# vitskvara/VBMatrixFactorization.jl

Hardware: AMD Instinct MI355X
Metric: VB iterations/sec (higher is better)
Workload: dtype bf16

## Files before the change

### include/vbmf_hip.h

```cpp
#ifndef VBMF_HIP_H
#define VBMF_HIP_H

#include <stddef.h>
#include <stdint.h>

#ifdef __cplusplus
extern "C" {
#endif

typedef struct vbmf_ctx vbmf_ctx;

typedef enum {
    VBMF_OK = 0,
    VBMF_ERR_INVALID = -1,
    VBMF_ERR_NO_DEVICE = -2,
    VBMF_ERR_HIP = -3,
    VBMF_ERR_NUMERIC = -4,
    VBMF_ERR_COMM = -5,
    VBMF_ERR_UNSUPPORTED = -6,
    VBMF_ERR_SYNC = -7
} vbmf_status;

#define VBMF_Y_F32 0
#define VBMF_Y_BF16 1
// ... 192 lines not shown
int vbmf_dual_set_priors(vbmf_ctx* ctx, int64_t H0, double alpha00, double beta00, double alpha01, double beta01,
                         double alpha0, double alpha1);
int vbmf_dual_get_priors(vbmf_ctx* ctx, int64_t* H0, double* priors6);
int vbmf_dual_run(vbmf_ctx* ctx, int64_t niter, double eps, int est_cb, int est_priors, int64_t* iters_done,
                  double* d_last, double* trace);

int vbmf_trial_set_priors(vbmf_ctx* ctx, int64_t H0, int64_t M0, const double* priors9);
int vbmf_trial_get_priors(vbmf_ctx* ctx, int64_t* H0, int64_t* M0, double* priors9);
int vbmf_trial_run(vbmf_ctx* ctx, int64_t niter, double eps, int est_cb, int est_priors, int64_t* iters_done,
                   double* d_last, double* trace);


typedef struct vbmf_prep vbmf_prep;
int vbmf_preprocess_open(vbmf_prep** out, int device, const double* Y, int64_t L, int64_t M, int64_t ldY, int64_t* L_used);
int vbmf_preprocess_rows(const vbmf_prep* plan, int64_t* used_rows0, double* mu, double* den);
int vbmf_set_Y_preprocessed(vbmf_ctx* ctx, const vbmf_prep* plan, double lambda);
int vbmf_preprocess_close(vbmf_prep* plan);

#define VBMF_UNIQUE_ID_BYTES 128
int vbmf_comm_unique_id(void* id128);
int vbmf_comm_init(vbmf_ctx* ctx, const void* id128);
typedef int (*vbmf_allreduce_fn)(void* user, void* buf, size_t count, int is_double, void* hip_stream);
int vbmf_comm_set_transport(vbmf_ctx* ctx, vbmf_allreduce_fn fn, void* user);

int vbmf_profile_enable(vbmf_ctx* ctx, int on);
int vbmf_profile_read(vbmf_ctx* ctx, double* out8, int reset);
int vbmf_pass_bytes(vbmf_ctx* ctx, int pass, double* bytes);
int vbmf_device_sync(vbmf_ctx* ctx);

#define VBMF_PEEK_P 0
#define VBMF_PEEK_Q 1
#define VBMF_PEEK_A32 2
#define VBMF_PEEK_B32 3
#define VBMF_PEEK_FA 4
#define VBMF_PEEK_FB 5
#define VBMF_PEEK_Y1 6
#define VBMF_PEEK_Y2 7
#define VBMF_PEEK_DIMS 8
#define VBMF_PEEK_CHAIN 9
#define VBMF_PEEK_STATE 10
#define VBMF_PEEK_GRAM_W 11
#define VBMF_PEEK_GRAM_PQ 12
#define VBMF_PEEK_GRAM_G 13
#define VBMF_PEEK_SA32 14
#define VBMF_PEEK_SB32 15
int vbmf_debug_peek(vbmf_ctx* ctx, int what, uint32_t* out, int64_t nwords, int64_t word_offset);
int vbmf_debug_time_pass(vbmf_ctx* ctx, int pass, int iters, double* ms);
#define VBMF_DEBUG_EPI_SPIN_LIMIT 0
#define VBMF_DEBUG_EPI_EXPECT_SKEW 1
#define VBMF_DEBUG_SIGMA_B_PPM 2
#define VBMF_DEBUG_EXACT_LAMBDA 3
int vbmf_debug_set(vbmf_ctx* ctx, int what, int64_t value);
int vbmf_debug_lambda_max(vbmf_ctx* ctx, const double* G, double* lambda_max, double* kernel_us);

#ifdef __cplusplus
}
#endif
#endif
```

### vbmatrixfactorization.jl_amd/capi.py

```python
import ctypes as C
import os

import numpy as np

_HERE = os.path.dirname(os.path.abspath(__file__))
LIB_PATH = os.environ.get("VBMF_HIP_LIB") or os.path.join(_HERE, "libvbmf_hip.so")
if os.environ.get("VBMF_HIP_LIB") and not os.path.isfile(LIB_PATH):
    raise FileNotFoundError(f"VBMF_HIP_LIB={LIB_PATH}: no such library (A/B variant builds: scripts/README.md)")

VBMF_Y_F32, VBMF_Y_BF16 = 0, 1
VBMF_SRC_F64, VBMF_SRC_F32, VBMF_SRC_BF16 = 0, 1, 2
VBMF_DST_F64, VBMF_DST_F32, VBMF_DST_BF16 = 0, 1, 2
VBMF_OUT_YHAT, VBMF_OUT_RESIDUAL = 0, 1
VBMF_FACTOR_A, VBMF_FACTOR_B = 0, 1
VBMF_FACTOR_AUTO, VBMF_FACTOR_BF16, VBMF_FACTOR_BF16X2 = 0, 1, 2
VBMF_FACTOR_BF16_MAX_H = 128
VBMF_VARIANT_BASIC, VBMF_VARIANT_SPARSE_DIAG, VBMF_VARIANT_SPARSE_DIAGVAR, VBMF_VARIANT_DUAL_DIAG, VBMF_VARIANT_TRIAL_DIAG = 0, 1, 2, 3, 4
VBMF_VARIANT_DUAL_DIAGVAR, VBMF_VARIANT_TRIAL_DIAGVAR = 5, 6
VBMF_COMPAT_SPECTRAL_DELTA, VBMF_COMPAT_SPARSE_REPEAT, VBMF_COMPAT_DEFAULT = 1, 2, 0xFFFFFFFF
STEP_A, STEP_B, STEP_CA, STEP_CB, STEP_SIGMA2 = 1, 2, 4, 8, 16
UNIQUE_ID_BYTES = 128
VBMF_FIT_FORM_STREAM, VBMF_FIT_FORM_GRAM, VBMF_FIT_FORM_AUTO = 0, 1, 2
VBMF_FIT_GRAM_WIDE_FACTOR = 2
VBMF_FIT_LDS_CAP_BYTES = 144 * 1024
# ... 10 lines not shown
        raise ValueError(f"form = {form!r} ('stream', 'gram' or 'auto')")
    return FIT_FORMS[form]


def ard_fit_form_code(form):
    if form == "gram":
        raise ValueError("form = 'gram': the ARD-sparse, two-group and three-group models have no Gram form (the element-wise precision "
                         "on A breaks A = Y'V); it serves the basic model's wide bags through vbmf_batch_")
    if not isinstance(form, str) or form not in ARD_FIT_FORMS:
        raise ValueError(f"form = {form!r} ('stream', 'split' or 'auto')")
    return ARD_FIT_FORMS[form]


def ard_slice_cols(slice_cols):
    sc = 0 if slice_cols is None else int(slice_cols)
    if sc != 0 and (sc < 8 or sc % 8):
        raise ValueError(f"slice_cols = {slice_cols!r} (None, or a multiple of 8)")
    return sc


def ard_fit_slices(Mb, slice_cols=None):
    sc = ard_slice_cols(slice_cols) or VBMF_FIT_SPLIT_COLS
    return -(-int(Mb) // sc)


def ard_fit_form_auto(Mb, full_cov=False):
    return VBMF_FIT_FORM_SPLIT if Mb >= (VBMF_FIT_SPLIT_MIN_COLS_FULL if full_cov else VBMF_FIT_SPLIT_MIN_COLS) else VBMF_FIT_FORM_STREAM


def fit_gram_fits(L, H):
    P = 16 if H <= 16 else 32
    return 3 * L * H <= VBMF_FIT_LDS_CAP_BYTES // 8 - (P * (P + 2) + 9 * H * H)


def fit_form_auto(L, Mb, H):
    return int(Mb >= VBMF_FIT_GRAM_WIDE_FACTOR * L and fit_gram_fits(L, H))

SYMBOLS = [
    "vbmf_default_opts", "vbmf_create", "vbmf_destroy", "vbmf_last_error", "vbmf_set_Y", "vbmf_set_Y_rows", "vbmf_set_Y_synthetic",
    "vbmf_get_Y", "vbmf_get_trYY", "vbmf_set_state", "vbmf_get_state", "vbmf_step", "vbmf_run", "vbmf_run_fixed_basis",
    "vbmf_run_fixed_basis_batched", "vbmf_fit_batched", "vbmf_fit_batched_form", "vbmf_bags_row_gram", "vbmf_get_YHat",
    "vbmf_elbo", "vbmf_comm_unique_id", "vbmf_comm_init", "vbmf_comm_set_transport", "vbmf_profile_enable", "vbmf_profile_read",
    "vbmf_pass_bytes", "vbmf_device_sync", "vbmf_debug_peek", "vbmf_debug_time_pass", "vbmf_debug_lambda_max",
    "vbmf_sparse_set_state", "vbmf_sparse_get_state", "vbmf_sparse_step", "vbmf_sparse_run", "vbmf_sparse_run_fixed_basis",
    "vbmf_sparse_run_fixed_basis_batched", "vbmf_sparse_fit_batched", "vbmf_local_fit_batched", "vbmf_rows_fit_batched",
    "vbmf_ard_fit_batched_form",
    "vbmf_sparse_lower_bound", "vbmf_sparse_set_noise_rows", "vbmf_sparse_get_noise_rows", "vbmf_preprocess_open", "vbmf_preprocess_rows", "vbmf_set_Y_preprocessed",
    "vbmf_preprocess_close", "vbmf_dual_set_priors", "vbmf_dual_get_priors", "vbmf_dual_run",
    "vbmf_trial_set_priors", "vbmf_trial_get_priors", "vbmf_trial_run",
    "vbmf_sparse_set_full_cov", "vbmf_sparse_set_SigmaA", "vbmf_sparse_get_SigmaA",
    "vbmf_sparse_lower_bound_trimmed", "vbmf_debug_set",
    "vbmf_bag_residuals", "vbmf_sparse_lower_bound_batched", "vbmf_bag_least_squares", "vbmf_bag_least_squares_jobs", "vbmf_set_gram_form",
    "vbmf_sparse_fixed_basis_jobs", "vbmf_debug_vbls_jobs_lds_cols",
    "vbmf_get_YHat_rows", "vbmf_get_factor_rows", "vbmf_set_Y_gather",
]
VBMF_OK, VBMF_ERR_INVALID, VBMF_ERR_NO_DEVICE, VBMF_ERR_HIP, VBMF_ERR_NUMERIC, VBMF_ERR_COMM, VBMF_ERR_UNSUPPORTED, VBMF_ERR_SYNC = 0, -1, -2, -3, -4, -5, -6, -7
DEBUG_EPI_SPIN_LIMIT, DEBUG_EPI_EXPECT_SKEW, DEBUG_SIGMA_B_PPM, DEBUG_EXACT_LAMBDA = 0, 1, 2, 3
SSTEP_A, SSTEP_B, SSTEP_CA, SSTEP_CB, SSTEP_SIGMA, SSTEP_PRIORS = 1, 2, 4, 8, 16, 32
(PEEK_P, PEEK_Q, PEEK_A32, PEEK_B32, PEEK_FA, PEEK_FB, PEEK_Y1, PEEK_Y2, PEEK_DIMS, PEEK_CHAIN, PEEK_STATE, PEEK_GRAM_W,
 PEEK_GRAM_PQ, PEEK_GRAM_G, PEEK_SA32, PEEK_SB32) = range(16)


class VbmfOpts(C.Structure):
    _fields_ = [
        ("struct_size", C.c_int32), ("device", C.c_int32), ("y_dtype", C.c_int32), ("factor_dtype", C.c_int32),
        ("variant", C.c_int32), ("reference_compat", C.c_uint32), ("nranks", C.c_int32), ("rank", C.c_int32),
        ("L_global", C.c_int64), ("row_offset", C.c_int64), ("pass1_splits", C.c_int32), ("reserved", C.c_int32),
    ]


class VbmfSparseHyper(C.Structure):
    _fields_ = [("alpha0", C.c_double), ("beta0", C.c_double), ("gamma0", C.c_double), ("delta0", C.c_double),
                ("eta0", C.c_double), ("zeta0", C.c_double)]


ALLREDUCE_FN = C.CFUNCTYPE(C.c_int, C.c_void_p, C.c_void_p, C.c_size_t, C.c_int, C.c_void_p)


class VbmfError(RuntimeError):
    def __init__(self, code, msg):
        super().__init__(f"vbmf_hip error {code}: {msg}")
        self.code = code


_lib = None


def lib():
    global _lib
    if _lib is not None:
        return _lib
    try:
        import torch
    except Exception:
        pass
    if not os.path.exists(LIB_PATH):
        raise ImportError(
            f"{LIB_PATH} is missing: build it with `python vbmatrixfactorization.jl_amd/build.py` "
            "(hipcc, gfx950).  This package has no CPU fallback.")
    L = C.CDLL(LIB_PATH, mode=C.RTLD_GLOBAL)
    dp, i64, i32, vp = C.POINTER(C.c_double), C.c_int64, C.c_int, C.c_void_p
    L.vbmf_default_opts.argtypes = [C.POINTER(VbmfOpts)]
    L.vbmf_default_opts.restype = None
    L.vbmf_create.argtypes = [C.POINTER(vp), i64, i64, i64, C.POINTER(VbmfOpts)]
    L.vbmf_destroy.argtypes = [vp]
    L.vbmf_last_error.argtypes = [vp]
    L.vbmf_last_error.restype = C.c_char_p
# ... 1 lines not shown
    L.vbmf_set_Y_rows.argtypes = [vp, vp, C.c_int32, C.c_int32, i64, i64, i64, i64]
    L.vbmf_set_Y_gather.argtypes = [vp, vp, C.POINTER(i64), i64]
    L.vbmf_set_Y_synthetic.argtypes = [vp, C.c_uint64, i64, C.c_double]
    L.vbmf_get_Y.argtypes = [vp, dp, i64, i64, i64]
    L.vbmf_get_trYY.argtypes = [vp, dp]
    L.vbmf_set_state.argtypes = [vp, dp, i64, dp, i64, dp, dp, dp, dp, C.c_double, C.POINTER(i64), i64, i64]
    L.vbmf_get_state.argtypes = [vp, dp, i64, dp, i64, dp, dp, dp, dp, dp]
    L.vbmf_step.argtypes = [vp, i32]
    L.vbmf_run.argtypes = [vp, i64, C.c_double, i32, i32, C.POINTER(i64), dp, dp]
    L.vbmf_run_fixed_basis.argtypes = [vp, i64]
    L.vbmf_run_fixed_basis_batched.argtypes = [vp, i64, C.POINTER(i64), i64, dp, dp, dp, dp, i64]
    L.vbmf_fit_batched.argtypes = ([vp, i64, C.POINTER(i64), i64, C.POINTER(i64), i64, C.c_double, i32, i32] + [dp] * 7
                                   + [C.POINTER(i64), dp, C.POINTER(i64), dp])
    L.vbmf_fit_batched_form.argtypes = L.vbmf_fit_batched.argtypes + [i64, C.POINTER(i64)]
    L.vbmf_bags_row_gram.argtypes = [vp, i64, C.POINTER(i64), dp]
    L.vbmf_sparse_run_fixed_basis.argtypes = [vp, i64]
    L.vbmf_sparse_run_fixed_basis_batched.argtypes = [vp, i64, C.POINTER(i64), i64, i32, dp, dp, dp, dp, dp, dp, dp, dp, dp, dp, dp]
    L.vbmf_sparse_fit_batched.argtypes = ([vp, i64, C.POINTER(i64), i64, C.POINTER(i64), i64, C.c_double, i32, i32, i32, i64] + [dp] * 16
                                          + [C.POINTER(i64), dp, C.POINTER(i64), dp])
    L.vbmf_local_fit_batched.argtypes = ([vp, i64, C.POINTER(i64), i64, C.POINTER(i64), i64, C.c_double, i32, i32, i32, i64,
                                          C.POINTER(i64), i64] + [dp] * 16 + [C.POINTER(i64), dp, C.POINTER(i64), dp])
    L.vbmf_rows_fit_batched.argtypes = L.vbmf_local_fit_batched.argtypes
    L.vbmf_ard_fit_batched_form.argtypes = L.vbmf_local_fit_batched.argtypes + [C.c_int, i64, i64, C.POINTER(i64)]
    L.vbmf_get_YHat.argtypes = [vp, dp, i64]
    L.vbmf_get_YHat_rows.argtypes = [vp, C.c_int32, vp, C.c_int32, C.c_int32, i64, i64, i64, i64]
    L.vbmf_get_factor_rows.argtypes = [vp, C.c_int32, vp, C.c_int32, C.c_int32, i64, i64, i64, i64]
    L.vbmf_elbo.argtypes = [vp, dp]
    L.vbmf_comm_unique_id.argtypes = [vp]
    L.vbmf_comm_init.argtypes = [vp, vp]
    L.vbmf_comm_set_transport.argtypes = [vp, ALLREDUCE_FN, vp]
    L.vbmf_profile_enable.argtypes = [vp, i32]
    L.vbmf_profile_read.argtypes = [vp, dp, i32]
    L.vbmf_pass_bytes.argtypes = [vp, i32, dp]
    L.vbmf_device_sync.argtypes = [vp]
    L.vbmf_debug_peek.argtypes = [vp, i32, C.POINTER(C.c_uint32), i64, i64]
    L.vbmf_debug_time_pass.argtypes = [vp, i32, i32, dp]
    L.vbmf_debug_lambda_max.argtypes = [vp, dp, dp, dp]
    L.vbmf_sparse_set_state.argtypes = [vp, dp, dp, dp, dp, dp, i64, dp, dp, dp, C.c_double, C.c_double,
                                        C.POINTER(VbmfSparseHyper), C.POINTER(i64), i64, i64]
    L.vbmf_sparse_get_state.argtypes = [vp, dp, dp, dp, dp, dp, dp, i64, dp, dp, dp, dp, dp]
    L.vbmf_sparse_step.argtypes = [vp, i32]
    L.vbmf_sparse_run.argtypes = [vp, i64, C.c_double, i32, C.POINTER(i64), dp, dp]
    L.vbmf_sparse_lower_bound.argtypes = [vp, i32, dp]
    L.vbmf_sparse_lower_bound_trimmed.argtypes = [vp, i32, C.c_double, dp]
    L.vbmf_debug_set.argtypes = [vp, i32, i64]
    L.vbmf_bag_residuals.argtypes = [vp, i64, C.POINTER(i64), dp, i64, dp]
    L.vbmf_sparse_lower_bound_batched.argtypes = [vp, i64, C.POINTER(i64), i32, C.c_double, i32] + [dp] * 15
    L.vbmf_bag_least_squares.argtypes = [vp, i64, C.POINTER(i64), dp, i64, i64, C.c_double, dp, i64, dp]
    L.vbmf_bag_least_squares_jobs.argtypes = [vp, i64, C.POINTER(i64), i64, C.POINTER(i64), dp, dp, i64, C.POINTER(i64), C.POINTER(i64), dp, dp,
                                              C.POINTER(i64)]
    L.vbmf_sparse_fixed_basis_jobs.argtypes = [vp, i64, C.POINTER(i64), i64, i64, i32, i64, dp, dp, dp, dp, dp, dp, dp, dp, i64,
                                               C.POINTER(i64), C.POINTER(i64), dp, dp, dp, dp, dp, dp, dp, dp, C.POINTER(i64)]
    L.vbmf_debug_vbls_jobs_lds_cols.argtypes = [i64, i32]
    L.vbmf_sparse_set_full_cov.argtypes = [vp, i32]
    L.vbmf_set_gram_form.argtypes = [vp, i32]
    L.vbmf_sparse_set_SigmaA.argtypes = [vp, dp]
    L.vbmf_sparse_get_SigmaA.argtypes = [vp, dp]
    L.vbmf_dual_set_priors.argtypes = [vp, i64] + [C.c_double] * 6
    L.vbmf_dual_get_priors.argtypes = [vp, C.POINTER(i64), dp]
    L.vbmf_dual_run.argtypes = [vp, i64, C.c_double, i32, i32, C.POINTER(i64), dp, dp]
    L.vbmf_trial_set_priors.argtypes = [vp, i64, i64, dp]
    L.vbmf_trial_get_priors.argtypes = [vp, C.POINTER(i64), C.POINTER(i64), dp]
    L.vbmf_trial_run.argtypes = [vp, i64, C.c_double, i32, i32, C.POINTER(i64), dp, dp]
    L.vbmf_sparse_set_noise_rows.argtypes = [vp, dp, dp, C.c_double]
    L.vbmf_sparse_get_noise_rows.argtypes = [vp, dp, dp]
    L.vbmf_preprocess_open.argtypes = [C.POINTER(vp), i32, dp, i64, i64, i64, C.POINTER(i64)]
    L.vbmf_preprocess_rows.argtypes = [vp, C.POINTER(i64), dp, dp]
    L.vbmf_set_Y_preprocessed.argtypes = [vp, vp, C.c_double]
    L.vbmf_preprocess_close.argtypes = [vp]
    for name in SYMBOLS:
        if name not in ("vbmf_default_opts", "vbmf_last_error"):
            getattr(L, name).restype = C.c_int
    _lib = L
    return L


def _dptr(a):
    return a.ctypes.data_as(C.POINTER(C.c_double)) if a is not None else None


def _i64ptr(a):
    return a.ctypes.data_as(C.POINTER(C.c_int64)) if a is not None else None


def _fcol(a, shape=None):
    a = np.asarray(a, dtype=np.float64)
    if shape is not None and tuple(a.shape) != tuple(shape):
        raise ValueError(f"expected shape {shape}, got {a.shape}")
    return np.asfortranarray(a)


def _is_tensor(a):
    return hasattr(a, "data_ptr") and hasattr(a, "is_cuda")


def y_source(src, device=0):
    if _is_tensor(src):
        import torch
        codes = {torch.float64: VBMF_SRC_F64, torch.float32: VBMF_SRC_F32, torch.bfloat16: VBMF_SRC_BF16}
        if src.dtype not in codes:
            raise TypeError(f"Y must be float64, float32 or bfloat16, got {src.dtype}")
        if src.dim() != 2:
            raise ValueError("Y must be a matrix")
        if src.is_cuda:
            if src.device.index != device:
                raise ValueError(f"Y lives on {src.device}, the context on GPU {device}")
# ... 662 lines not shown
        out = np.zeros(8)
        self._chk(self._lib.vbmf_profile_read(self._h, _dptr(out), int(reset)))
        return dict(pass1_ms=out[0], pass1_n=int(out[1]), pass2_ms=out[2], pass2_n=int(out[3]))

    def pass_bytes(self, p):
        v = C.c_double()
        self._chk(self._lib.vbmf_pass_bytes(self._h, p, C.byref(v)))
        return v.value

    def peek(self, what, nwords, offset=0, dtype=np.uint32):
        out = np.zeros(nwords, dtype=np.uint32)
        self._chk(self._lib.vbmf_debug_peek(self._h, what, out.ctypes.data_as(C.POINTER(C.c_uint32)), nwords, offset))
        return out.view(dtype)

    def chain_us(self):
        v = self.peek(PEEK_CHAIN, 16, dtype=np.uint64)
        return dict(zip(("ctrl_end", "SigmaA", "lambda_max_dB_and_loop", "SigmaB", "epilogue_table", "epilogue_tiles", "epilogue_fold"),
                        (float(x) * 0.01 for x in v)))

    def dims(self):
        v = self.peek(PEEK_DIMS, 30, dtype=np.int32)
        keys = ["Hp", "NH", "mode", "XT1", "KS1", "nsplit1", "sps1", "XT2", "KS2", "nsplit2", "sps2", "kstep", "npart", "narrow",
                "streamk_per", "streamk_grid",
                "gram", "gram_built", "gram_build_us", "gram_nsplit",
                "p_frag", "q_frag", "q_epi",
                "lds8", "xcd_map", "post3",
                "sparse_a_fused",
                "set_y_rows_us",
                "b_pending", "b_materialised"]
        return dict(zip(keys, (int(x) for x in v)))

    def out_rows_us(self):
        return int(self.peek(PEEK_DIMS, 31, dtype=np.int32)[30])

    def time_pass(self, p, iters=10):
        v = C.c_double()
        self._chk(self._lib.vbmf_debug_time_pass(self._h, p, iters, C.byref(v)))
        return v.value

    def lambda_max(self, G):
        G = np.asfortranarray(G, dtype=np.float64)
        assert G.shape == (self.H, self.H)
        v, us = C.c_double(), C.c_double()
        self._chk(self._lib.vbmf_debug_lambda_max(self._h, _dptr(G), C.byref(v), C.byref(us)))
        return v.value, us.value

    def sync(self):
        self._chk(self._lib.vbmf_device_sync(self._h))

    def debug_set(self, what, value):
        self._chk(self._lib.vbmf_debug_set(self._h, int(what), int(value)))


def vbls_jobs_lds_cols(H, full_cov=False):
    return int(lib().vbmf_debug_vbls_jobs_lds_cols(int(H), int(bool(full_cov))))
```

### vbmatrixfactorization.jl_amd/csrc/blk_inverse.hpp

```cpp
#pragma once
#include "common.hpp"

namespace vbmf {

typedef __attribute__((ext_vector_type(4))) double f64x4;

__device__ __forceinline__ double blk_rcp(double x) {
    double r = __builtin_amdgcn_rcp(x);
    r = fma(fma(-x, r, 1.0), r, r);
    r = fma(fma(-x, r, 1.0), r, r);
    return r;
}

template <int K>
__device__ __forceinline__ double row_bcast16(double v) {
    const int lo = __builtin_amdgcn_mov_dpp(__double2loint(v), 0x150 + K, 0xf, 0xf, false);
    const int hi = __builtin_amdgcn_mov_dpp(__double2hiint(v), 0x150 + K, 0xf, 0xf, false);
    return __hiloint2double(hi, lo);
}
template <int Q0>
__device__ __forceinline__ unsigned rows_bcast_u32(unsigned x) {
    const auto p = __builtin_amdgcn_permlane16_swap(x, x, false, false);
    const unsigned y = (Q0 & 1) ? p[1] : p[0];
    const auto s = __builtin_amdgcn_permlane32_swap(y, y, false, false);
// ... 41 lines not shown
    if constexpr (KK < 15) un = bperm_f64(rowaddr[Q1], a[R1]);
    double v[4];
#pragma unroll
    for (int r = 0; r < 4; ++r) v[r] = row_bcast16<KK>(a[r]);
    const double d = row_bcast16<KK>(u);
    pv.push(d);
    if (pivout != nullptr && c == 0 && q == 0) pivout[KK] = d;
    const double dinv = blk_rcp(d);
    const bool is_col = (c == KK), is_row = (q == Q0);
    const double w = is_col ? -dinv : u * dinv;
    v[R0] = is_row ? -1.0 : v[R0];
#pragma unroll
    for (int r = 0; r < 4; ++r) a[r] = fma(-v[r], w, zero_if(is_col || (r == R0 && is_row), a[r]));
    if constexpr (KK < 15) {
        const double vk1 = row_bcast16<KK>(un);
        u = fma(-vk1, w, zero_if(is_col, un));
    }
}
__device__ __forceinline__ void sweep16(f64x4& a, int lane, PivAcc& pv, double* pivout = nullptr) {
    const int c = lane & 15, q = lane >> 4;
    const int rowaddr[4] = {4 * c, 4 * (16 + c), 4 * (32 + c), 4 * (48 + c)};
    double u = bperm_f64(rowaddr[0], a[0]);
    sweep16_step<0>(a, u, c, q, rowaddr, pv, pivout);  sweep16_step<1>(a, u, c, q, rowaddr, pv, pivout);  sweep16_step<2>(a, u, c, q, rowaddr, pv, pivout);
    sweep16_step<3>(a, u, c, q, rowaddr, pv, pivout);  sweep16_step<4>(a, u, c, q, rowaddr, pv, pivout);  sweep16_step<5>(a, u, c, q, rowaddr, pv, pivout);
    sweep16_step<6>(a, u, c, q, rowaddr, pv, pivout);  sweep16_step<7>(a, u, c, q, rowaddr, pv, pivout);  sweep16_step<8>(a, u, c, q, rowaddr, pv, pivout);
    sweep16_step<9>(a, u, c, q, rowaddr, pv, pivout);  sweep16_step<10>(a, u, c, q, rowaddr, pv, pivout); sweep16_step<11>(a, u, c, q, rowaddr, pv, pivout);
    sweep16_step<12>(a, u, c, q, rowaddr, pv, pivout); sweep16_step<13>(a, u, c, q, rowaddr, pv, pivout); sweep16_step<14>(a, u, c, q, rowaddr, pv, pivout);
    sweep16_step<15>(a, u, c, q, rowaddr, pv, pivout);
    pv.fold();
}

__device__ __forceinline__ f64x4 blk_ld_rows(const double* W, int ld, int bi, int bj, int lane) {
    const double* p = W + (16 * bi + (lane >> 4)) * ld + 16 * bj + (lane & 15);
    return f64x4{p[0], p[4 * ld], p[8 * ld], p[12 * ld]};
}
__device__ __forceinline__ f64x4 blk_ld_cols(const double* W, int ld, int bi, int bj, int lane) {
    const double* p = W + (16 * bi + (lane & 15)) * ld + 16 * bj + (lane >> 4);
    return f64x4{p[0], p[4], p[8], p[12]};
}
__device__ __forceinline__ void blk_st_rows(double* W, int ld, int bi, int bj, int lane, const f64x4& x) {
    double* p = W + (16 * bi + (lane >> 4)) * ld + 16 * bj + (lane & 15);
    p[0] = x[0]; p[4 * ld] = x[1]; p[8 * ld] = x[2]; p[12 * ld] = x[3];
}
__device__ __forceinline__ void blk_st_cols(double* W, int ld, int bi, int bj, int lane, const f64x4& x) {
    double* p = W + (16 * bi + (lane & 15)) * ld + 16 * bj + (lane >> 4);
    p[0] = x[0]; p[4] = x[1]; p[8] = x[2]; p[12] = x[3];
}
__device__ __forceinline__ f64x4 blk_mma(const f64x4& a, const f64x4& b, f64x4 acc) {
#pragma unroll
    for (int kk = 0; kk < 4; ++kk) acc = __builtin_amdgcn_mfma_f64_16x16x4f64(a[kk], b[kk], acc, 0, 0, 0);
    return acc;
}

template <int NB, int NW>
__device__ __forceinline__ void blk_sweep(double* W, int ld, int nb_used, int w, int lane, PivAcc& pv) {
    for (int K = 0; K < nb_used; ++K) {
        f64x4 S = blk_ld_rows(W, ld, K, K, lane);
        sweep16(S, lane, pv);
        const f64x4 Sn = -S;
        f64x4 R[NB];
#pragma unroll
        for (int J = 0; J < NB; ++J) {
            if (J >= nb_used || J == K) continue;
            const f64x4 b = J > K ? blk_ld_rows(W, ld, K, J, lane) : blk_ld_cols(W, ld, J, K, lane);
            R[J] = blk_mma(Sn, b, f64x4{0.0, 0.0, 0.0, 0.0});
        }
        int pairno = 0;
#pragma unroll
        for (int I = 0; I < NB; ++I) {
            if (I >= nb_used || I == K) continue;
            f64x4 T = I < K ? blk_ld_cols(W, ld, I, K, lane) : blk_ld_rows(W, ld, K, I, lane);
            T = -T;
#pragma unroll
            for (int J = I; J < NB; ++J) {
                if (J >= nb_used || J == K) continue;
                if (NW == 1 || (pairno % NW) == w) {
                    f64x4 C = blk_ld_rows(W, ld, I, J, lane);
                    C = blk_mma(T, R[J], C);
                    blk_st_rows(W, ld, I, J, lane, C);
                }
                ++pairno;
            }
        }
        if constexpr (NW > 1) __syncthreads();
        if (NW == 1 || w == 0) {
#pragma unroll
            for (int J = 0; J < NB; ++J) {
                if (J >= nb_used || J == K) continue;
                if (J > K) blk_st_rows(W, ld, K, J, lane, R[J]);
                else blk_st_cols(W, ld, J, K, lane, R[J]);
            }
            blk_st_rows(W, ld, K, K, lane, S);
        }
        if constexpr (NW > 1) __syncthreads();
    }
}

constexpr int INV256_LD = 258;
constexpr int INV256_LDS_DOUBLES = 2 * 16 * INV256_LD + 16 * 18;
__device__ __forceinline__ void inv256_blk(const double* __restrict__ Kg, double* __restrict__ Out, double* lds, double* pivs, int nb = 16) {
    constexpr int LD = INV256_LD, NBLK = 136, NOWN = 9;
    double* Tst = lds;
    double* Rst = lds + 16 * LD;
    double* Sb = lds + 2 * 16 * LD;
    const int lane = threadIdx.x & 63;
    const int w = __builtin_amdgcn_readfirstlane(threadIdx.x >> 6);
    int bi[NOWN], bj[NOWN];
    f64x4 blk[NOWN];
// ... 7 lines not shown
        bj[t] = have ? I + (p - start) : -1;
        blk[t] = f64x4{0.0, 0.0, 0.0, 0.0};
        if (have) blk[t] = blk_ld_rows(Kg, 256, bi[t], bj[t], lane);
    }
    for (int K = 0; K < nb; ++K) {
#pragma unroll
        for (int t = 0; t < NOWN; ++t) {
            if (bi[t] < 0) continue;
            if (bi[t] == K && bj[t] == K) {
                PivAcc pv;
                sweep16(blk[t], lane, pv, pivs + 16 * K);
                blk_st_rows(Sb, 18, 0, 0, lane, -blk[t]);
            } else if (bi[t] == K) {
                blk_st_rows(Tst, LD, 0, bj[t], lane, blk[t]);
            } else if (bj[t] == K) {
                blk_st_cols(Tst, LD, 0, bi[t], lane, blk[t]);
            }
        }
        __syncthreads();
        const f64x4 Sn = blk_ld_rows(Sb, 18, 0, 0, lane);
#pragma unroll
        for (int t = 0; t < NOWN; ++t) {
            if (bi[t] < 0 || (bi[t] == K) == (bj[t] == K)) continue;
            const int J = bi[t] == K ? bj[t] : bi[t];
            const f64x4 b = blk_ld_rows(Tst, LD, 0, J, lane);
            const f64x4 R = blk_mma(Sn, b, f64x4{0.0, 0.0, 0.0, 0.0});
            blk_st_rows(Rst, LD, 0, J, lane, R);
            if (bi[t] == K) blk[t] = R;
        }
        __syncthreads();
#pragma unroll
        for (int t = 0; t < NOWN; ++t) {
            if (bi[t] < 0) continue;
            if (bi[t] != K && bj[t] != K) {
                const f64x4 T = -blk_ld_rows(Tst, LD, 0, bi[t], lane);
                const f64x4 Rj = blk_ld_rows(Rst, LD, 0, bj[t], lane);
                blk[t] = blk_mma(T, Rj, blk[t]);
            } else if (bj[t] == K && bi[t] != K) {
                blk[t] = blk_ld_cols(Rst, LD, 0, bi[t], lane);
            }
        }
        __syncthreads();
    }
#pragma unroll
    for (int t = 0; t < NOWN; ++t) {
        if (bi[t] < 0) continue;
        const f64x4 v = -blk[t];
        blk_st_rows(Out, 256, bi[t], bj[t], lane, v);
        if (bi[t] != bj[t]) blk_st_cols(Out, 256, bj[t], bi[t], lane, v);
    }
    __syncthreads();
}

}
```

### vbmatrixfactorization.jl_amd/csrc/vbmf_hip.hip

```cpp
#include "../../include/vbmf_hip.h"

#include <hip/hip_runtime.h>
#include <rccl/rccl.h>

#include <algorithm>
#include <chrono>
#include <cmath>
#include <cstdio>
#include <cstring>
#include <string>
#include <thread>
#include <type_traits>
#include <vector>

#include "common.hpp"
#include "ctx_cache.hpp"
#include "ctx_mem.hpp"
#include "ctrl_kernels.hpp"
#include "post_kernels.hpp"
#include "rng.hpp"
#include "sparse_kernels.hpp"
#include "stream_gemm.hpp"
#include "tile_kernels.hpp"
#include "prep_kernels.hpp"
// ... 2135 lines not shown
    HIPCHK(c, hipGetLastError());
    return VBMF_OK;
}
static int launch_yhat_out(vbmf_ctx* c, int what, void* dev, int dt, int64_t l0, int64_t n, int64_t rs, int64_t cs) {
    if (dt == VBMF_DST_F64) return launch_yhat_typed<double, double>(c, what, (double*)dev, l0, n, rs, cs);
    if (dt == VBMF_DST_F32) return launch_yhat_typed<float, float>(c, what, (float*)dev, l0, n, rs, cs);
    return launch_yhat_typed<float, out_bf16>(c, what, (out_bf16*)dev, l0, n, rs, cs);
}
static int launch_factor_out(vbmf_ctx* c, const float* F, void* dev, int dt, int64_t x0, int64_t n, int64_t rs, int64_t cs) {
    const int grid = grid_for(n * c->H), hfast = cs <= rs;
#define VBMF_FAC_LAUNCH(T)                                                                                                  \
    hipLaunchKernelGGL((factor_out_kernel<T>), dim3(grid), dim3(256), 0, c->stream, F, c->Hp, (int)c->H, (long long)x0, \
                       (long long)n, (T*)dev, (long long)rs, (long long)cs, hfast)
    if (dt == VBMF_DST_F64) VBMF_FAC_LAUNCH(double);
    else if (dt == VBMF_DST_F32) VBMF_FAC_LAUNCH(float);
    else VBMF_FAC_LAUNCH(out_bf16);
#undef VBMF_FAC_LAUNCH
    HIPCHK(c, hipGetLastError());
    return VBMF_OK;
}

template <class Emit>
static int write_block(vbmf_ctx* c, const char* fn, void* dst, int dt, int on_device, int64_t row0, int64_t nrows, int64_t ncols,
                       int64_t rs, int64_t cs, Emit emit) {
    const size_t es = dst_elem_size(dt);
    if (!c->ev_y[0]) { HIPCHK(c, hipEventCreate(&c->ev_y[0])); HIPCHK(c, hipEventCreate(&c->ev_y[1])); }
    HIPCHK(c, hipEventRecord(c->ev_y[0], c->stream));
    if (on_device) {
        TRY(emit(dst, row0, nrows, rs, cs));
    } else {
        const bool rowmajor = cs == 1 && (nrows == 1 || rs >= ncols);
        int64_t rc = std::max<int64_t>(1, (int64_t)(256ll << 20) / (ncols * (int64_t)es));
        rc = std::min(rc, nrows);
        DevScratch<void> stage;
        MEMCHK(c, stage.alloc((size_t)rc * ncols * es));
        for (int64_t r = 0; r < nrows; r += rc) {
            const int64_t n = std::min(rc, nrows - r);
            TRY(rowmajor ? emit(stage.get(), row0 + r, n, ncols, (int64_t)1) : emit(stage.get(), row0 + r, n, (int64_t)1, n));
            char* to = (char*)dst + (size_t)r * rs * es;
            hipError_t e = rowmajor ? hipMemcpy2DAsync(to, (size_t)rs * es, stage, (size_t)ncols * es, (size_t)ncols * es, (size_t)n, hipMemcpyDeviceToHost, c->stream)
                                    : hipMemcpy2DAsync(to, (size_t)cs * es, stage, (size_t)n * es, (size_t)n * es, (size_t)ncols, hipMemcpyDeviceToHost, c->stream);
            if (e == hipSuccess) e = hipStreamSynchronize(c->stream);
            if (e != hipSuccess) FAIL(c, VBMF_ERR_HIP, "%s: copy to the host failed: %s", fn, hipGetErrorString(e));
        }
    }
    HIPCHK(c, hipEventRecord(c->ev_y[1], c->stream));
    HIPCHK(c, hipStreamSynchronize(c->stream));
    float ms = 0.0f;
    HIPCHK(c, hipEventElapsedTime(&ms, c->ev_y[0], c->ev_y[1]));
    c->out_ms = ms;
    return VBMF_OK;
}

extern "C" {

int vbmf_get_YHat_rows(vbmf_ctx* c, int32_t what, void* dst, int32_t dt, int32_t on_device, int64_t row0, int64_t nrows,
                       int64_t rs, int64_t cs) {
    if (!c) return VBMF_ERR_INVALID;
    static const char* fn = "vbmf_get_YHat_rows";
    if (!dst) FAIL(c, VBMF_ERR_INVALID, "%s: null dst", fn);
    if (what != VBMF_OUT_YHAT && what != VBMF_OUT_RESIDUAL) FAIL(c, VBMF_ERR_INVALID, "%s: unknown what %d", fn, (int)what);
    TRY(check_dst(c, fn, dst, dt, on_device, row0, nrows, c->L, c->M, rs, cs));
    if (!c->cache.have_state()) FAIL(c, VBMF_ERR_INVALID, "%s: no state", fn);
    if (what == VBMF_OUT_RESIDUAL && !c->cache.have_Y()) FAIL(c, VBMF_ERR_INVALID, "%s: no Y", fn);
    TRY(ensure_B(c));
    TRY(rebuild_B32_if_stale(c));
    return write_block(c, fn, dst, dt, on_device, row0, nrows, c->M, rs, cs,
                       [&](void* dev, int64_t l0, int64_t n, int64_t r, int64_t s) { return launch_yhat_out(c, what, dev, dt, l0, n, r, s); });
}

int vbmf_get_factor_rows(vbmf_ctx* c, int32_t which, void* dst, int32_t dt, int32_t on_device, int64_t row0, int64_t nrows,
                         int64_t rs, int64_t cs) {
    if (!c) return VBMF_ERR_INVALID;
    static const char* fn = "vbmf_get_factor_rows";
    if (!dst) FAIL(c, VBMF_ERR_INVALID, "%s: null dst", fn);
    if (which != VBMF_FACTOR_A && which != VBMF_FACTOR_B) FAIL(c, VBMF_ERR_INVALID, "%s: unknown which %d", fn, (int)which);
    TRY(check_dst(c, fn, dst, dt, on_device, row0, nrows, which == VBMF_FACTOR_A ? c->M : c->L, c->H, rs, cs));
    if (!c->cache.have_state()) FAIL(c, VBMF_ERR_INVALID, "%s: no state", fn);
    if (which == VBMF_FACTOR_B) {
        TRY(ensure_B(c));
        TRY(rebuild_B32_if_stale(c));
    }
    return write_block(c, fn, dst, dt, on_device, row0, nrows, c->H, rs, cs, [&](void* dev, int64_t x0, int64_t n, int64_t r, int64_t s) {
        return launch_factor_out(c, which == VBMF_FACTOR_A ? c->A32 : c->B32[c->bcur], dev, dt, x0, n, r, s);
    });
}

int vbmf_elbo(vbmf_ctx* c, double* elbo) {
    if (!c || !elbo) return VBMF_ERR_INVALID;
    HIPCHK(c, hipSetDevice(c->o.device));
    TRY(ensure_ready(c));
    TRY(ensure_gram_A(c));
    TRY(ensure_gram_B(c));
    int f = 0;
    TRY(prepare_trYBA(c, &f));
    TRY(launch_ctrl_end(c, f, 0.0, nullptr));
    HIPCHK(c, hipMemcpyAsync(c->scal_host, c->st + c->lay.scal(), 32 * 8, hipMemcpyDeviceToHost, c->stream));
    HIPCHK(c, hipStreamSynchronize(c->stream));
    *elbo = c->scal_host[S_ELBO];
    return VBMF_OK;
}

int vbmf_comm_unique_id(void* id128) {
    if (!id128) return VBMF_ERR_INVALID;
    static_assert(sizeof(ncclUniqueId) <= VBMF_UNIQUE_ID_BYTES, "unique id size");
    ncclUniqueId id;
// ... 111 lines not shown
}

int vbmf_debug_time_pass(vbmf_ctx* c, int pass, int iters, double* ms) {
    if (!c || !ms || (pass != 1 && pass != 2) || iters < 1) return VBMF_ERR_INVALID;
    HIPCHK(c, hipSetDevice(c->o.device));
    TRY(ensure_ready(c));
    hipEvent_t a, b;
    HIPCHK(c, hipEventCreate(&a));
    HIPCHK(c, hipEventCreate(&b));
    const int prof = c->prof;
    c->prof = 0;
    int rc = launch_stream(c, pass - 1);
    if (rc == VBMF_OK) rc = launch_stream(c, pass - 1);
    hipEventRecord(a, c->stream);
    for (int i = 0; i < iters && rc == VBMF_OK; ++i) rc = launch_stream(c, pass - 1);
    hipEventRecord(b, c->stream);
    hipEventSynchronize(b);
    float t = 0.f;
    hipEventElapsedTime(&t, a, b);
    hipEventDestroy(a);
    hipEventDestroy(b);
    c->prof = prof;
    c->cache.P_overwritten();
    *ms = t / iters;
    return rc;
}

int vbmf_debug_lambda_max(vbmf_ctx* c, const double* G, double* lam, double* kernel_us) {
    if (!c || !G || !lam) return VBMF_ERR_INVALID;
    HIPCHK(c, hipSetDevice(c->o.device));
    TRY(ensure_B(c));
    const int H = (int)c->H, Hp = c->Hp;
    std::vector<double> g((size_t)Hp * Hp, 0.0);
    for (int j = 0; j < H; ++j)
        for (int i = 0; i < H; ++i) g[(size_t)i * Hp + j] = G[(size_t)j * H + i];
    HIPCHK(c, hipMemcpyAsync(c->st + c->lay.GD(), g.data(), g.size() * sizeof(double), hipMemcpyHostToDevice, c->stream));
    HIPCHK(c, hipMemsetAsync(c->ints + I_STOP, 0, sizeof(int), c->stream));
    hipEvent_t a, b;
    HIPCHK(c, hipEventCreate(&a));
    HIPCHK(c, hipEventCreate(&b));
    hipEventRecord(a, c->stream);
    int rc = launch_eig(c, 1, 0);
    hipEventRecord(b, c->stream);
    hipEventSynchronize(b);
    float t = 0.f;
    hipEventElapsedTime(&t, a, b);
    hipEventDestroy(a);
    hipEventDestroy(b);
    if (rc != VBMF_OK) return rc;
    HIPCHK(c, hipMemcpyAsync(lam, c->st + c->lay.scal() + S_LAMD, sizeof(double), hipMemcpyDeviceToHost, c->stream));
    HIPCHK(c, hipStreamSynchronize(c->stream));
    if (kernel_us) *kernel_us = 1e3 * (double)t;
    return VBMF_OK;
}

int vbmf_debug_set(vbmf_ctx* c, int what, int64_t value) {
    if (!c) return VBMF_ERR_INVALID;
    HIPCHK(c, hipSetDevice(c->o.device));
    TRY(ensure_B(c));
    switch (what) {
        case VBMF_DEBUG_EXACT_LAMBDA:
            c->exact_lambda = value != 0;
            return VBMF_OK;
        case VBMF_DEBUG_EPI_SPIN_LIMIT:
            if (value < 1 || value > (1ll << 30)) FAIL(c, VBMF_ERR_INVALID, "vbmf_debug_set: spin limit out of range");
            c->epi_spin_limit = (int)value;
            return VBMF_OK;
        case VBMF_DEBUG_EPI_EXPECT_SKEW:
            c->epi_expect_skew = value ? 1 : 0;
            return VBMF_OK;
        case VBMF_DEBUG_SIGMA_B_PPM: {
            if (value < -1000000 || value > 1000000) FAIL(c, VBMF_ERR_INVALID, "vbmf_debug_set: ppm out of range");
            c->dbg_sb_ppm = (int)value;
            HIPCHK(c, hipSetDevice(c->o.device));
            HIPCHK(c, memcpy_sync(c, c->ints + I_DBG_SB_PPM, &c->dbg_sb_ppm, sizeof(int), hipMemcpyHostToDevice));
            return VBMF_OK;
        }
        default: FAIL(c, VBMF_ERR_INVALID, "vbmf_debug_set: unknown knob");
    }
}

int vbmf_device_sync(vbmf_ctx* c) {
    if (!c) return VBMF_ERR_INVALID;
    HIPCHK(c, hipSetDevice(c->o.device));
    HIPCHK(c, hipStreamSynchronize(c->stream));
    return VBMF_OK;
}


}

static double digamma_host(double x) {
    double r = 0.0;
    while (x < 10.0) { r -= 1.0 / x; x += 1.0; }
    const double f = 1.0 / (x * x);
    return r + std::log(x) - 0.5 / x -
           f * (1.0 / 12 - f * (1.0 / 120 - f * (1.0 / 252 - f * (1.0 / 240 - f * (5.0 / 660 - f * (691.0 / 32760))))));
}

static int launch_sparse_cov_b(vbmf_ctx* c) {
    ctrl_tier(c->H, [&](auto r, auto t) {
        constexpr int R = decltype(r)::value, T = decltype(t)::value;
        hipLaunchKernelGGL((sparse_cov_b_kernel<R, T>), dim3(1), dim3(T * T), (cov_lds_bytes<R, T>()), ctrl_stream(c), c->st, c->lay, (int)c->H,
                           c->SB32, c->ints, c->diagvar ? 1 : 0);
    });
    HIPCHK(c, hipGetLastError());
// ... 780 lines not shown
```

Baseline: 4741.

## Add look-ahead blocked sweep overlapping next pivot with bulk updates

For small block counts with multiple waves, the blocked sweep inverse now dedicates one wave to the critical path: it sweeps the diagonal block and precomputes the next pivot block early. The remaining waves perform the trailing Schur updates in parallel. This aims to shorten the serialized pivot chain per block step, at the cost of more complex mirror-indexing logic and extra barriers on the last step. A debug entry point for testing the sweep in isolation is also added.

```diff
diff --git a/include/vbmf_hip.h b/include/vbmf_hip.h
--- a/include/vbmf_hip.h
+++ b/include/vbmf_hip.h
@@ -268,6 +268,7 @@
 #define VBMF_DEBUG_EXACT_LAMBDA 3
 int vbmf_debug_set(vbmf_ctx* ctx, int what, int64_t value);
 int vbmf_debug_lambda_max(vbmf_ctx* ctx, const double* G, double* lambda_max, double* kernel_us);
+int vbmf_debug_blk_sweep(const double* K, int64_t H, int waves, double* out, double* logdet, int* bad);
 
 #ifdef __cplusplus
 }
diff --git a/vbmatrixfactorization.jl_amd/capi.py b/vbmatrixfactorization.jl_amd/capi.py
--- a/vbmatrixfactorization.jl_amd/capi.py
+++ b/vbmatrixfactorization.jl_amd/capi.py
@@ -86,7 +86,7 @@
     "vbmf_sparse_lower_bound_trimmed", "vbmf_debug_set",
     "vbmf_bag_residuals", "vbmf_sparse_lower_bound_batched", "vbmf_bag_least_squares", "vbmf_bag_least_squares_jobs", "vbmf_set_gram_form",
     "vbmf_sparse_fixed_basis_jobs", "vbmf_debug_vbls_jobs_lds_cols",
-    "vbmf_get_YHat_rows", "vbmf_get_factor_rows", "vbmf_set_Y_gather",
+    "vbmf_get_YHat_rows", "vbmf_get_factor_rows", "vbmf_set_Y_gather", "vbmf_debug_blk_sweep",
 ]
 VBMF_OK, VBMF_ERR_INVALID, VBMF_ERR_NO_DEVICE, VBMF_ERR_HIP, VBMF_ERR_NUMERIC, VBMF_ERR_COMM, VBMF_ERR_UNSUPPORTED, VBMF_ERR_SYNC = 0, -1, -2, -3, -4, -5, -6, -7
 DEBUG_EPI_SPIN_LIMIT, DEBUG_EPI_EXPECT_SKEW, DEBUG_SIGMA_B_PPM, DEBUG_EXACT_LAMBDA = 0, 1, 2, 3
@@ -194,6 +194,7 @@
     L.vbmf_sparse_fixed_basis_jobs.argtypes = [vp, i64, C.POINTER(i64), i64, i64, i32, i64, dp, dp, dp, dp, dp, dp, dp, dp, i64,
                                                C.POINTER(i64), C.POINTER(i64), dp, dp, dp, dp, dp, dp, dp, dp, C.POINTER(i64)]
     L.vbmf_debug_vbls_jobs_lds_cols.argtypes = [i64, i32]
+    L.vbmf_debug_blk_sweep.argtypes = [dp, i64, i32, dp, dp, C.POINTER(i32)]
     L.vbmf_sparse_set_full_cov.argtypes = [vp, i32]
     L.vbmf_set_gram_form.argtypes = [vp, i32]
     L.vbmf_sparse_set_SigmaA.argtypes = [vp, dp]
@@ -962,5 +963,18 @@
         self._chk(self._lib.vbmf_debug_set(self._h, int(what), int(value)))
 
 
+def blk_sweep(K, waves=4):
+    K = np.ascontiguousarray(K, dtype=np.float64)
+    H = K.shape[0]
+    assert K.shape == (H, H)
+    n = 16 * ((H + 15) // 16)
+    out = np.empty((n, n), dtype=np.float64)
+    ld, bad = C.c_double(), C.c_int32()
+    rc = lib().vbmf_debug_blk_sweep(_dptr(K), H, int(waves), _dptr(out), C.byref(ld), C.byref(bad))
+    if rc != VBMF_OK:
+        raise RuntimeError("vbmf_debug_blk_sweep failed: %d" % rc)
+    return out, ld.value, bad.value
+
+
 def vbls_jobs_lds_cols(H, full_cov=False):
     return int(lib().vbmf_debug_vbls_jobs_lds_cols(int(H), int(bool(full_cov))))
diff --git a/vbmatrixfactorization.jl_amd/csrc/blk_inverse.hpp b/vbmatrixfactorization.jl_amd/csrc/blk_inverse.hpp
--- a/vbmatrixfactorization.jl_amd/csrc/blk_inverse.hpp
+++ b/vbmatrixfactorization.jl_amd/csrc/blk_inverse.hpp
@@ -117,8 +117,85 @@
     return acc;
 }
 
+__device__ __forceinline__ bool blk_in_mirror(int I, int J, int K) {
+    return I == K - 1 || (J == K - 1 && I != K - 2);
+}
+__device__ __forceinline__ f64x4 blk_ld_at(const double* W, int ld, int I, int J, int lane, bool mir) {
+    return mir ? blk_ld_cols(W, ld, J, I, lane) : blk_ld_rows(W, ld, I, J, lane);
+}
+__device__ __forceinline__ f64x4 blk_ld_at_t(const double* W, int ld, int I, int J, int lane, bool mir) {
+    return mir ? blk_ld_rows(W, ld, J, I, lane) : blk_ld_cols(W, ld, I, J, lane);
+}
+template <int NB, int NW>
+__device__ __forceinline__ void blk_sweep_ahead(double* W, int ld, int nb_used, int w, int lane, PivAcc& pv) {
+    static_assert(NW > 1, "one critical wave and at least one bulk wave");
+    f64x4 D = {0.0, 0.0, 0.0, 0.0};
+    if (w == 0) D = blk_ld_rows(W, ld, 0, 0, lane);
+    for (int K = 0; K < nb_used; ++K) {
+        const bool last = K == nb_used - 1;
+        if (w == 0) {
+            sweep16(D, lane, pv);
+            blk_st_rows(W, ld, K, K, lane, D);
+        }
+        __syncthreads();
+        if (w == 0 && !last) {
+            const f64x4 b = blk_ld_rows(W, ld, K, K + 1, lane);
+            const f64x4 R = blk_mma(-D, b, f64x4{0.0, 0.0, 0.0, 0.0});
+            D = blk_mma(-b, R, blk_ld_rows(W, ld, K + 1, K + 1, lane));
+        } else if (w != 0 || last) {
+            const int nbulk = last ? NW : NW - 1, me = last ? w : w - 1;
+            const f64x4 Sn = -blk_ld_rows(W, ld, K, K, lane);
+            f64x4 b[NB], R[NB];
+#pragma unroll
+            for (int J = 0; J < NB; ++J) {
+                if (J >= nb_used || J == K) continue;
+                b[J] = J > K ? blk_ld_rows(W, ld, K, J, lane) : blk_ld_at_t(W, ld, J, K, lane, J == K - 1);
+                R[J] = blk_mma(Sn, b[J], f64x4{0.0, 0.0, 0.0, 0.0});
+            }
+            int pairno = 0;
+#pragma unroll
+            for (int I = 0; I < NB; ++I) {
+                if (I >= nb_used || I == K) continue;
+                const f64x4 T = -b[I];
+#pragma unroll
+                for (int J = I; J < NB; ++J) {
+                    if (J >= nb_used || J == K) continue;
+                    if (I == K + 1 && J == K + 1) continue;
+                    if (pairno % nbulk == me) {
+                        f64x4 C = I == J ? blk_ld_rows(W, ld, I, I, lane) : blk_ld_at(W, ld, I, J, lane, blk_in_mirror(I, J, K));
+                        C = blk_mma(T, R[J], C);
+                        blk_st_rows(W, ld, I, J, lane, C);
+                    }
+                    ++pairno;
+                }
+            }
+            if (!last) {
+#pragma unroll
+                for (int J = 0; J < NB; ++J) {
+                    if (J >= nb_used || J == K || J % nbulk != me) continue;
+                    if (J > K) blk_st_cols(W, ld, J, K, lane, R[J]);
+                    else if (J == K - 1) blk_st_cols(W, ld, J, K, lane, R[J]);
+                    else blk_st_rows(W, ld, K, J, lane, R[J]);
+                }
+            } else {
+                __syncthreads();
+#pragma unroll
+                for (int J = 0; J < NB; ++J) {
+                    if (J >= nb_used || J == K || J % nbulk != me) continue;
+                    blk_st_cols(W, ld, J, K, lane, R[J]);
+                }
+                __syncthreads();
+            }
+        }
+    }
+}
+
 template <int NB, int NW>
 __device__ __forceinline__ void blk_sweep(double* W, int ld, int nb_used, int w, int lane, PivAcc& pv) {
+    if constexpr (NW > 1 && NB <= 4) {
+        blk_sweep_ahead<NB, NW>(W, ld, nb_used, w, lane, pv);
+        return;
+    }
     for (int K = 0; K < nb_used; ++K) {
         f64x4 S = blk_ld_rows(W, ld, K, K, lane);
         sweep16(S, lane, pv);
@@ -232,4 +309,31 @@
     __syncthreads();
 }
 
-}
+template <int NB, int NW>
+__global__ __launch_bounds__(256) void debug_blk_sweep_kernel(const double* __restrict__ Kg, int H, double* __restrict__ out,
+                                                              double* __restrict__ logdet, int* __restrict__ bad) {
+    extern __shared__ __attribute__((aligned(16))) double lds_dbs[];
+    constexpr int NP = 16 * NB, LD = NP + 2;
+    double* W = lds_dbs;
+    const int lane = threadIdx.x & 63, w = __builtin_amdgcn_readfirstlane(threadIdx.x >> 6);
+    const int nbu = (H + 15) >> 4, n = 16 * nbu;
+    for (int t = threadIdx.x; t < NP * NP; t += 256) {
+        const int i = t / NP, j = t % NP;
+        W[i * LD + j] = (i < H && j < H) ? Kg[(long long)i * H + j] : (i == j ? 1.0 : 0.0);
+    }
+    __syncthreads();
+    PivAcc pv;
+    if constexpr (NW == 1) {
+        if (w == 0) blk_sweep<NB, 1>(W, LD, nbu, 0, lane, pv);
+    } else {
+        blk_sweep<NB, NW>(W, LD, nbu, w, lane, pv);
+    }
+    __syncthreads();
+    for (int t = threadIdx.x; t < n * n; t += 256) {
+        const int i = t / n, j = t % n;
+        out[t] = (i >> 4) <= (j >> 4) ? W[i * LD + j] : 0.0;
+    }
+    if (threadIdx.x == 0) { *logdet = pv.logdet(); *bad = pv.bad; }
+}
+
+}
diff --git a/vbmatrixfactorization.jl_amd/csrc/vbmf_hip.hip b/vbmatrixfactorization.jl_amd/csrc/vbmf_hip.hip
--- a/vbmatrixfactorization.jl_amd/csrc/vbmf_hip.hip
+++ b/vbmatrixfactorization.jl_amd/csrc/vbmf_hip.hip
@@ -2211,6 +2211,17 @@
     return VBMF_OK;
 }
 
+template <int NB>
+static hipError_t debug_blk_sweep_launch(int waves, const double* dK, int H, double* dOut, double* dLd, int* dBad) {
+    const void* fn = waves == 1 ? (const void*)debug_blk_sweep_kernel<NB, 1> : (const void*)debug_blk_sweep_kernel<NB, 4>;
+    const size_t lds = spd_inverse_lds_bytes(NB);
+    hipError_t e = hipFuncSetAttribute(fn, hipFuncAttributeMaxDynamicSharedMemorySize, (int)lds);
+    if (e != hipSuccess) return e;
+    if (waves == 1) hipLaunchKernelGGL((debug_blk_sweep_kernel<NB, 1>), dim3(1), dim3(256), lds, 0, dK, H, dOut, dLd, dBad);
+    else hipLaunchKernelGGL((debug_blk_sweep_kernel<NB, 4>), dim3(1), dim3(256), lds, 0, dK, H, dOut, dLd, dBad);
+    return hipGetLastError();
+}
+
 extern "C" {
 
 int vbmf_get_YHat_rows(vbmf_ctx* c, int32_t what, void* dst, int32_t dt, int32_t on_device, int64_t row0, int64_t nrows,
@@ -2428,6 +2439,29 @@
     HIPCHK(c, hipStreamSynchronize(c->stream));
     if (kernel_us) *kernel_us = 1e3 * (double)t;
     return VBMF_OK;
+}
+
+int vbmf_debug_blk_sweep(const double* K, int64_t H, int waves, double* out, double* logdet, int* bad) {
+    if (!K || !out || !logdet || !bad || H < 1 || H > 128 || (waves != 1 && waves != 4)) return VBMF_ERR_INVALID;
+    const int h = (int)H, n = 16 * ((h + 15) >> 4);
+    const size_t kb = (size_t)h * h * sizeof(double), ob = (size_t)n * n * sizeof(double);
+    double* d = nullptr;
+    if (hipMalloc(&d, kb + ob + 2 * sizeof(double)) != hipSuccess) return VBMF_ERR_HIP;
+    double* dOut = d + (size_t)h * h;
+    double* dLd = dOut + (size_t)n * n;
+    int* dBad = reinterpret_cast<int*>(dLd + 1);
+    hipError_t e = hipMemcpy(d, K, kb, hipMemcpyHostToDevice);
+    if (e == hipSuccess)
+        e = h <= 16 ? debug_blk_sweep_launch<1>(waves, d, h, dOut, dLd, dBad)
+          : h <= 32 ? debug_blk_sweep_launch<2>(waves, d, h, dOut, dLd, dBad)
+          : h <= 64 ? debug_blk_sweep_launch<4>(waves, d, h, dOut, dLd, dBad)
+                    : debug_blk_sweep_launch<8>(waves, d, h, dOut, dLd, dBad);
+    if (e == hipSuccess) e = hipDeviceSynchronize();
+    if (e == hipSuccess) e = hipMemcpy(out, dOut, ob, hipMemcpyDeviceToHost);
+    if (e == hipSuccess) e = hipMemcpy(logdet, dLd, sizeof(double), hipMemcpyDeviceToHost);
+    if (e == hipSuccess) e = hipMemcpy(bad, dBad, sizeof(int), hipMemcpyDeviceToHost);
+    hipFree(d);
+    return e == hipSuccess ? VBMF_OK : VBMF_ERR_HIP;
 }
 
 int vbmf_debug_set(vbmf_ctx* c, int what, int64_t value) {
```

After: 4817, median of 6. 1.02x the previous value.
